# NightShade99/Self-Supervised-Vision

Hardware: AMD Instinct MI355X
Metric: images/sec (whole node) SimCLR ResNet-50 two-view train step (higher is better)
Workload: dtype f32; 1 GPU; SimCLR resnet50 (7x7/2 stem) synthetic 3x224x224, bs=512/GPU, global batch 512, NT-Xent(normalize, T=0.5) over the global batch, SGD-Nesterov; per_gpu_batch=512, global_batch=512, params=27971008, parallelism=single, view_streams=2, library=self-supervised-vision_amd/csrc/libssv_hip.so

## Files before the change

### include/ssv_hip.h

```cpp
#ifndef SSV_HIP_H
#define SSV_HIP_H

#include <stddef.h>
#include <stdint.h>

#ifdef __cplusplus
extern "C" {
#endif

typedef enum ssv_status {
  SSV_OK = 0,
  SSV_ERR_INVALID = -1,
  SSV_ERR_WORKSPACE = -2,
  SSV_ERR_LAUNCH = -3
} ssv_status;

int ssv_version(void);
const char* ssv_last_error(void);
const char* ssv_source_sha16(void);
int ssv_device_cus(void);

typedef struct ssv_conv_desc {
  int32_t N, H, W, C;
  int32_t K, R, S;
  int32_t stride, pad;
  int32_t Ho, Wo;
  int32_t arithmetic;
  int32_t reserved;
  const void* w_planes;
} ssv_conv_desc;
enum { SSV_ARITH_F32_MFMA = 0, SSV_ARITH_BF16X3 = 6 };
int ssv_conv_arithmetic(const ssv_conv_desc* d, int32_t product);
int ssv_split_planes(int64_t n, const float* x, void* planes, void* stream);

int ssv_conv2d_fwd(const ssv_conv_desc* d, const float* x, const float* w, const float* bias,
                   const float* addend, float* y, void* stream);
int ssv_pad_channels(int64_t npix, int32_t cin, int32_t cout, const float* in, float* out, int32_t accumulate, void* stream);
int ssv_group_expand(int32_t K, int32_t R, int32_t S, int32_t Cg, int32_t groups, const float* wg, float* wd, void* stream);
int ssv_group_extract(int32_t K, int32_t R, int32_t S, int32_t Cg, int32_t groups, const float* dwd, float* dwg, int32_t accumulate, void* stream);

int ssv_conv2d_fwd_grouped(const ssv_conv_desc* d, int32_t groups, const float* x, const float* wd, const float* bias, const float* addend,
                           float* y, void* stream);
int ssv_conv2d_dgrad_grouped(const ssv_conv_desc* d, int32_t groups, const float* dy, const float* wd, const float* addend, float* dx, void* stream);
size_t ssv_conv2d_wgrad_grouped_workspace_bytes(const ssv_conv_desc* d, int32_t groups);
int ssv_conv2d_wgrad_grouped(const ssv_conv_desc* d, int32_t groups, const float* x, const float* dy, float* dwd, int accumulate,
                             void* ws, size_t ws_bytes, void* stream);
int ssv_filter_transpose(int32_t K, int32_t R, int32_t S, int32_t C, const float* w, float* wt, void* stream);
int64_t ssv_conv2d_fwd_stats_groups(const ssv_conv_desc* d);
int ssv_conv2d_fwd_stats(const ssv_conv_desc* d, const float* x, const float* w, float* y, float* pmean, float* pm2, void* stream);
int ssv_conv2d_fwd_bnrelu_in_stats(const ssv_conv_desc* d, const float* x, const float* in_scale, const float* in_shift,
                                   const float* w, float* y, float* pmean, float* pm2, void* stream);
int ssv_conv2d_wgrad_bnrelu_in(const ssv_conv_desc* d, const float* x, const float* in_scale, const float* in_shift, const float* dy,
                               float* dw, int accumulate, void* ws, size_t ws_bytes, void* stream);
typedef struct ssv_bn_gate {
  const float* x;
  const float* scale;
  const float* shift;
  const uint8_t* mask;
  const float* mean;
  const float* invstd;
  float* psum_g;
  float* psum_gx;
  const float* x2;
  const float* mean2;
  const float* invstd2;
  float* psum_gx2;
} ssv_bn_gate;
int64_t ssv_conv2d_fwd_gate_groups(const ssv_conv_desc* d);
int ssv_conv2d_fwd_gated(const ssv_conv_desc* d, const float* x, const float* w, const float* addend, float* y,
                         const ssv_bn_gate* gate, void* stream);
typedef struct ssv_bn_dyin {
  const float* x;
  const float* coef;
} ssv_bn_dyin;
int ssv_conv2d_fwd_dyin(const ssv_conv_desc* d, const float* g, const ssv_bn_dyin* dyin, const float* w, const float* addend, float* y,
                        const ssv_bn_gate* gate, void* stream);
int ssv_conv2d_wgrad_dyin(const ssv_conv_desc* d, const float* x, const float* in_scale, const float* in_shift, const float* g,
                          const ssv_bn_dyin* dyin, float* dw, int accumulate, void* ws, size_t ws_bytes, void* stream);
int ssv_conv2d_fwd_sumin_stats(const ssv_conv_desc* d, const float* x, const float* res, const float* scale, const float* shift,
                               const float* rscale, const float* rshift, const float* w, float* y, float* pmean, float* pm2,
                               float* a_out, uint8_t* mask_out, void* stream);
int ssv_conv2d_fwd_gated_s2add(const ssv_conv_desc* d, const float* x, const float* w, const float* addend, int32_t H2, int32_t W2, float* y,
                               const ssv_bn_gate* gate, void* stream);
int ssv_conv2d_fwd_dyin_s2add(const ssv_conv_desc* d, const float* g, const ssv_bn_dyin* dyin, const float* w, const float* addend,
// ... 344 lines not shown
```

### self-supervised-vision_amd/csrc/conv_mfma.hip

```cpp
#include "common.h"
#include "split_bf16.h"
#include <string.h>
#include <type_traits>

namespace {

constexpr int GBK = 16;

__device__ __forceinline__ int xcd_remap(int orig, int nwg) {
  const int q = nwg >> 3, r = nwg & 7, xcd = orig & 7;
  return (xcd < r ? xcd * (q + 1) : r * (q + 1) + (xcd - r) * q) + (orig >> 3);
}

struct ConvKP {
  int N, H, W, C, K, R, S, stride, pad, Ho, Wo;
  int M;
  int RSC;
  FastDiv dHoWo, dWo, dC, dS, dWp;
  float* aux_out;
  float* aux_out2;
  const float* aux_in;
  const float* xf_scale;
  const float* xf_shift;
  ssv_bn_gate gate;
  const float* dyin_x;
  const float* dyin_coef;
  const float* sum_res; const float* sum_scale; const float* sum_shift; const float* sum_rscale; const float* sum_rshift;
  float* sum_out; uint8_t* sum_mask;
  long long bs_a, bs_b, bs_o;
  int add_H2, add_W2;
  int Cg, Kg;
  const unsigned short* w_planes;
  long long wp_stride;
};

__device__ __forceinline__ void group_span(int n0, int n1, int og, int ig, int bk, int ctot, int& lo, int& hi) {
  const int glo = n0 / og, ghi = (n1 - 1) / og;
  lo = glo * ig / bk * bk;
  hi = min(ctot, ((ghi + 1) * ig + bk - 1) / bk * bk);
}

constexpr int XF_MAXC = 1024;

__device__ __forceinline__ float gelu_f(float v) { return ssv_gelu(v); }
__device__ __forceinline__ float gelu_grad_f(float v) { return ssv_gelu_grad(v); }

using rsrc_t = __amdgpu_buffer_rsrc_t;
constexpr int OOB_OFF = (int)0x80000000u;
__device__ __forceinline__ rsrc_t make_rsrc(const void* base, unsigned bytes) {
  return __builtin_amdgcn_make_buffer_rsrc((void*)base, 0, bytes, 0x00020000);
}
__device__ __forceinline__ f32x4 bload4(rsrc_t rs, int voff_bytes, int soff_bytes) {
  typedef unsigned int u32x4_ __attribute__((ext_vector_type(4)));
  return __builtin_bit_cast(f32x4, (u32x4_)__builtin_amdgcn_raw_buffer_load_b128(rs, voff_bytes, soff_bytes, 0));
}

__device__ __forceinline__ int straddle_off(int off, int bytes, int& rot) {
  rot = 0;
  if (off == OOB_OFF) return OOB_OFF;
  if (off <= -16 || off >= bytes) return OOB_OFF;
  const int c = off < 0 ? 0 : (off > bytes - 16 ? bytes - 16 : off);
  rot = (off - c) >> 2;
  return c;
}
__device__ __forceinline__ f32x4 straddle_fix(f32x4 v, int rot) {
  f32x4 o;
#pragma unroll
  for (int e = 0; e < 4; ++e) {
    const int sidx = e + rot;
    float t = 0.f;
#pragma unroll
// ... 169 lines not shown
      for (int j = 0; j < TN16; ++j) lo[i][j] = f32x4{0.f, 0.f, 0.f, 0.f};
  }
  load_tile();
  xform_tile();
  store_tile();
  __syncthreads();
  for (int kt = 0; kt < nkt; ++kt) {
    load_tile();
    constexpr int TJ = TN16 / JSPLIT;
    static_assert(TN16 % JSPLIT == 0, "column tiles per group");
#pragma unroll
    for (int jg = 0; jg < JSPLIT; ++jg) {
      bf16x8 fb[TJ][3];
#pragma unroll
      for (int j = 0; j < TJ; ++j)
#pragma unroll
        for (int q = 0; q < 3; ++q) {
          if constexpr (KROWB) fb[j][q] = splitbf::krow_frag<RBB>(Bs + q * b_plane, wc0 + 16 * (jg * TJ + j), lane);
          else fb[j][q] = splitbf::rowk_frag(Bs + q * b_plane, wc0 + 16 * (jg * TJ + j), lane);
        }
#pragma unroll
      for (int i = 0; i < TM16; ++i) {
        bf16x8 fa[3];
#pragma unroll
        for (int q = 0; q < 3; ++q) {
          if constexpr (KROWA) fa[q] = splitbf::krow_frag<RBA>(As + q * a_plane, wr0 + 16 * i, lane);
          else fa[q] = splitbf::rowk_frag(As + q * a_plane, wr0 + 16 * i, lane);
        }
#pragma unroll
        for (int j = 0; j < TJ; ++j) {
          if constexpr (DUAL) splitbf::mma6x2(acc[i][jg * TJ + j], lo[i][jg * TJ + j], fb[j], fa);
          else splitbf::mma6(acc[i][jg * TJ + j], fb[j], fa);
        }
      }
    }
    if constexpr (FLUSH > 0) {
      if ((kt + 1) % FLUSH == 0) {
#pragma unroll
        for (int i = 0; i < TM16; ++i)
#pragma unroll
          for (int j = 0; j < TN16; ++j) { hi[i][j] += acc[i][j]; acc[i][j] = f32x4{0.f, 0.f, 0.f, 0.f}; }
      }
    }
    __syncthreads();
    if (kt + 1 < nkt) { xform_tile(); store_tile(); __syncthreads(); }
  }
#pragma unroll
  for (int i = 0; i < TM16; ++i)
#pragma unroll
    for (int j = 0; j < TN16; ++j) {
      if constexpr (FLUSH > 0) acc[i][j] = hi[i][j] + acc[i][j];
      if constexpr (DUAL) acc[i][j] += lo[i][j];
    }
}

__device__ __forceinline__ void bstore4(rsrc_t rs, int voff_bytes, f32x4 v) {
  typedef unsigned int u32x4_ __attribute__((ext_vector_type(4)));
  __builtin_amdgcn_raw_buffer_store_b128(__builtin_bit_cast(u32x4_, v), rs, voff_bytes, 0, 0);
}

struct SameOff {};
template <int TM, int TN>
__device__ __forceinline__ void stage_slab(const f32x16 (&acc)[TM][TN], float* __restrict__ ep, int tm, int lane) {
  constexpr int LDE = TN * 32 + 4;
  const int l31 = lane & 31, h = lane >> 5;
#pragma unroll
  for (int tn = 0; tn < TN; ++tn)
#pragma unroll
    for (int j = 0; j < 16; ++j) ep[((j & 3) + 8 * (j >> 2) + 4 * h) * LDE + tn * 32 + l31] = acc[tm][tn][j];
}
template <int TM, int TN>
__device__ __forceinline__ void stage_slab(const f32x4 (&acc)[2 * TM][2 * TN], float* __restrict__ ep, int tm, int lane) {
  constexpr int LDE = TN * 32 + 4;
  const int fr = lane & 15, kg = lane >> 4;
#pragma unroll
  for (int ii = 0; ii < 2; ++ii)
#pragma unroll
    for (int jj = 0; jj < 2 * TN; ++jj) *reinterpret_cast<f32x4*>(&ep[(16 * ii + fr) * LDE + 16 * jj + 4 * kg]) = acc[2 * tm + ii][jj];
}
template <bool SP, class A, class B> __device__ __forceinline__ auto& sel_acc(A& a, B& b) { if constexpr (SP) return b; else return a; }

template <int TM, int TN, int EPI = 0, bool STATS = false, int GATE = 0, class Acc, class RowOff, class AddOff = SameOff>
__device__ __forceinline__ void epilogue_vec(const Acc& acc, float* __restrict__ ep, int lane, int col0, int ncols,
                                             const float* __restrict__ bias, const float* addend, float* out, long long out_elems, RowOff&& row_off,
                                             float* out_act = nullptr, const float* gate = nullptr,
                                             float* pmean = nullptr, float* pm2 = nullptr, int group_rows = 0,
                                             const ssv_bn_gate* bn = nullptr, long long group = 0, AddOff add_off = AddOff(), long long add_elems = 0) {
  constexpr int LDE = TN * 32 + 4, C4 = TN * 8, RPI = 64 / C4, NP = 32 / RPI;
  constexpr bool GMASK = GATE >= 2, GX2 = GATE == 3;
  constexpr int HB0 = GATE == 1 ? 2 : 4;
  constexpr int HB = NP < HB0 ? NP : HB0;
  const int r_in = lane / C4, c4 = lane % C4;
  const int gcol = col0 + c4 * 4;
  const bool cok = gcol < ncols && r_in < RPI;
  const unsigned bytes = (unsigned)(out_elems * 4);
  const rsrc_t r_out = make_rsrc(out, bytes);
  f32x4 b4 = {0.f, 0.f, 0.f, 0.f};
  f32x4 st_p = {0.f, 0.f, 0.f, 0.f}, st_s1 = {0.f, 0.f, 0.f, 0.f}, st_s2 = {0.f, 0.f, 0.f, 0.f};
  f32x4 g_mu = {0.f, 0.f, 0.f, 0.f}, g_is = {0.f, 0.f, 0.f, 0.f}, g_sc = {0.f, 0.f, 0.f, 0.f}, g_sh = {0.f, 0.f, 0.f, 0.f};
  f32x4 g_mu2 = {0.f, 0.f, 0.f, 0.f}, g_is2 = {0.f, 0.f, 0.f, 0.f}, st_s3 = {0.f, 0.f, 0.f, 0.f};
  if constexpr (GATE != 0) {
    if (cok) {
      g_mu = *reinterpret_cast<const f32x4*>(bn->mean + gcol); g_is = *reinterpret_cast<const f32x4*>(bn->invstd + gcol);
      if constexpr (GATE == 1) { g_sc = *reinterpret_cast<const f32x4*>(bn->scale + gcol); g_sh = *reinterpret_cast<const f32x4*>(bn->shift + gcol); }
      if constexpr (GX2) { g_mu2 = *reinterpret_cast<const f32x4*>(bn->mean2 + gcol); g_is2 = *reinterpret_cast<const f32x4*>(bn->invstd2 + gcol); }
    }
// ... 86 lines not shown
          }
          bstore4(r_out, voff[sl][i], v);
          if constexpr (EPI == 1) {
            f32x4 a;
#pragma unroll
            for (int e = 0; e < 4; ++e) a[e] = gelu_f(v[e]);
            bstore4(r_act, voff[sl][i], a);
          }
        }
      };
      {
#pragma unroll
        for (int st = 0; st < NSTEP; ++st) {
          __builtin_amdgcn_sched_barrier(0);
          issue(st, 0);
          finish(st, 0);
        }
      }
    }
  };
  if constexpr (GATE != 0 || EPI == 2 || EPI == 5) rows(std::integral_constant<int, 2>{});
  else if (ADD) rows(std::integral_constant<int, 1>{});
  else rows(std::integral_constant<int, 0>{});

  if constexpr (STATS) {
#pragma unroll
    for (int o = C4; o < 64; o <<= 1) {
#pragma unroll
      for (int e = 0; e < 4; ++e) { st_s1[e] += __shfl_xor(st_s1[e], o, 64); st_s2[e] += __shfl_xor(st_s2[e], o, 64); }
    }
    if (r_in == 0 && cok && group_rows > 0) {
      const float n = (float)group_rows;
      *reinterpret_cast<f32x4*>(pmean + gcol) = st_p + st_s1 / n;
      *reinterpret_cast<f32x4*>(pm2 + gcol) = st_s2 - st_s1 * st_s1 / n;
    }
  }
  if constexpr (GATE != 0) {
#pragma unroll
    for (int o = C4; o < 64; o <<= 1) {
#pragma unroll
      for (int e = 0; e < 4; ++e) {
        st_s1[e] += __shfl_xor(st_s1[e], o, 64); st_s2[e] += __shfl_xor(st_s2[e], o, 64);
        if constexpr (GX2) st_s3[e] += __shfl_xor(st_s3[e], o, 64);
      }
    }
    if (r_in == 0 && cok) {
      *reinterpret_cast<f32x4*>(bn->psum_g + group * ncols + gcol) = st_s1;
      *reinterpret_cast<f32x4*>(bn->psum_gx + group * ncols + gcol) = st_s2;
      if constexpr (GX2) *reinterpret_cast<f32x4*>(bn->psum_gx2 + group * ncols + gcol) = st_s3;
    }
  }
}

template <int BM, int BN, int WGM, int WGN, int BK, bool VEC, int EPI = 0, bool STATS = false, int C4 = 0, bool XF = false, int GATE = 0, int OPM = 0, bool ADDS2 = false, int SP = 0>
__global__ void __launch_bounds__(256, (SP ? (OPM != 0 || GATE == 3 || (SP == 2 && BN == 128))
                                          : (OPM == 2 || GATE == 3 || (OPM == 1 && !(BM == 128 && BN == 128)))) ? 2 : 3)
conv_fwd_k(ConvKP p, const float* __restrict__ x, const float* __restrict__ w, const float* __restrict__ bias,
           const float* addend, float* y) {
  constexpr int TM = BM / WGM / 32, TN = BN / WGN / 32;
  constexpr int LDT = BK + 4;
  constexpr int STAGE = (BM + BN) * LDT;
  static_assert(!XF || (VEC && C4 == 0), "the fused-input variant is the float4 path");
  constexpr bool DYF = OPM == 1, SUM = OPM == 2;
  static_assert(OPM == 0 || (VEC && C4 == 0 && !XF), "the formed-on-load operands are the float4 path");
  constexpr int EP_FLOATS = 4 * 32 * (TN * 32 + 4);
  static_assert(!SP || (VEC && C4 == 0 && BK == 32), "the bf16-piece variants are the float4 path with K-step 32");
  constexpr int SP_FLOATS = (BM + BN) * 48;
  constexpr int SMEM = SP ? (SP_FLOATS > EP_FLOATS ? SP_FLOATS : EP_FLOATS)
                          : ((VEC && (EPI || STATS || GATE != 0 || OPM != 0) && EP_FLOATS > STAGE) ? EP_FLOATS : STAGE);
  __shared__ __attribute__((aligned(16))) float smem[SMEM];
  __shared__ __attribute__((aligned(16))) float xfs[(XF && !SP) ? 2 * XF_MAXC : 4];
  float* As = smem;
  float* Bs = smem + BM * LDT;
  const int tid = threadIdx.x, lane = tid & 63, wave = tid >> 6;
  const int wr0 = (wave / WGN) * (BM / WGM), wc0 = (wave % WGN) * (BN / WGN);
  const int NT = (p.K + BN - 1) / BN;
  const int bid = xcd_remap(blockIdx.x, gridDim.x);
  const int mt = bid / NT, nt = bid - mt * NT;
  const int m0 = mt * BM, n0 = nt * BN;
  x += (size_t)blockIdx.y * p.bs_a; w += (size_t)blockIdx.y * p.bs_b; y += (size_t)blockIdx.y * p.bs_o;
  if (addend) addend += (size_t)blockIdx.y * p.bs_o;

  f32x16 acc[SP ? 1 : TM][SP ? 1 : TN];
  f32x4 acc16[SP ? 2 * TM : 1][SP ? 2 * TN : 1];
  if constexpr (SP) {
#pragma unroll
    for (int i = 0; i < 2 * TM; ++i)
#pragma unroll
      for (int j = 0; j < 2 * TN; ++j) acc16[i][j] = f32x4{0.f, 0.f, 0.f, 0.f};
  } else zero_acc<SP ? 1 : TM, SP ? 1 : TN>(acc);

  if constexpr (VEC && C4 == 2) {
    static_assert(BK == 24 && BM == 256, "one staged output row per thread, six float4 per row");
    constexpr int CHN = BK / 4;
    constexpr int BF = (BN * CHN + 255) / 256;
    const rsrc_t rx = make_rsrc(x, (unsigned)p.N * p.H * p.W * 12u);
    const rsrc_t rw = make_rsrc(w, (unsigned)p.K * p.R * BK * 4u);
    int hi0, rowbase;
    unsigned wmask = 0;
    {
      const int m = m0 + tid;
      const bool ok = m < p.M;
      const uint32_t mm = ok ? (uint32_t)m : 0u;
      const uint32_t n = fdiv(mm, p.dHoWo);
      const uint32_t rem = mm - n * (uint32_t)(p.Ho * p.Wo);
      const uint32_t ho = fdiv(rem, p.dWo);
      const uint32_t wo = rem - ho * (uint32_t)p.Wo;
      hi0 = ok ? (int)ho * p.stride - p.pad : -(1 << 20);
      const int wi0 = (int)wo * p.stride - p.pad;
      rowbase = ok ? (((int)n * p.H + hi0) * p.W + wi0) * 12 : 0;
#pragma unroll
      for (int px = 0; px < 8; ++px) wmask |= (unsigned)((px < p.S) & ((unsigned)(wi0 + px) < (unsigned)p.W)) << px;
    }
    int boff[BF];
#pragma unroll
    for (int i = 0; i < BF; ++i) {
      const int f = tid + 256 * i, kf = f / CHN, ch = f - kf * CHN;
      boff[i] = (f < BN * CHN && n0 + kf < p.K) ? ((n0 + kf) * p.R * BK + ch * 4) * 4 : OOB_OFF;
    }
    int lr = 0;
// ... 34 lines not shown
      }
    };
    k_loop<TM, TN, true, true, LDT, LDT, BK, CHN + BF>(p.R, As, Bs, wr0, wc0, lane, acc, load_tile, store_tile, xform_tile);
  } else if constexpr (VEC && C4 == 1) {
    constexpr int CH = BK / 4, RPP = 256 / CH;
    constexpr int AP = BM / RPP, BP = BN / RPP;
    const int tl = tid % CH, rsub = tid / CH;
    const rsrc_t rx = make_rsrc(x, (unsigned)p.N * p.H * p.W * 16u);
    const rsrc_t rw = make_rsrc(w, (unsigned)p.K * p.RSC * 4u);
    int hi0[AP], wi0[AP], aoff[AP];
#pragma unroll
    for (int i = 0; i < AP; ++i) {
      const int m = m0 + rsub + RPP * i;
      const bool ok = m < p.M;
      const uint32_t mm = ok ? (uint32_t)m : 0u;
      const uint32_t n = fdiv(mm, p.dHoWo);
      const uint32_t rem = mm - n * (uint32_t)(p.Ho * p.Wo);
      const uint32_t ho = fdiv(rem, p.dWo);
      const uint32_t wo = rem - ho * (uint32_t)p.Wo;
      hi0[i] = ok ? (int)ho * p.stride - p.pad : -(1 << 20);
      wi0[i] = (int)wo * p.stride - p.pad;
      aoff[i] = (((int)n * p.H + hi0[i]) * p.W + wi0[i]) * 16;
    }
    int boff[BP];
#pragma unroll
    for (int i = 0; i < BP; ++i) {
      const int ko = n0 + rsub + RPP * i;
      boff[i] = ko < p.K ? ko * p.RSC * 4 : OOB_OFF;
    }
    const int ntap = p.R * p.S;
    int lt = tl;
    f32x4 ra[AP], rb[BP];
    auto load_tile = [&]() {
      const bool tv = lt < ntap;
      const int r = (int)fdiv((uint32_t)(tv ? lt : 0), p.dS);
      const int sx = (tv ? lt : 0) - r * p.S;
      const int toff_x = (r * p.W + sx) * 16, toff_w = lt * 16;
#pragma unroll
      for (int i = 0; i < AP; ++i) {
        const bool ok = tv & ((unsigned)(hi0[i] + r) < (unsigned)p.H) & ((unsigned)(wi0[i] + sx) < (unsigned)p.W);
        ra[i] = bload4(rx, ok ? aoff[i] + toff_x : OOB_OFF, 0);
      }
#pragma unroll
      for (int i = 0; i < BP; ++i) rb[i] = bload4(rw, (tv && boff[i] != OOB_OFF) ? boff[i] + toff_w : OOB_OFF, 0);
      lt += CH;
    };
    auto store_tile = [&]() {
#pragma unroll
      for (int i = 0; i < AP; ++i) *reinterpret_cast<f32x4*>(&As[(rsub + RPP * i) * LDT + tl * 4]) = ra[i];
#pragma unroll
      for (int i = 0; i < BP; ++i) *reinterpret_cast<f32x4*>(&Bs[(rsub + RPP * i) * LDT + tl * 4]) = rb[i];
    };
    k_loop<TM, TN, true, true, LDT, LDT, BK, AP + BP>((ntap + CH - 1) / CH, As, Bs, wr0, wc0, lane, acc, load_tile, store_tile);
  } else if constexpr (VEC) {
    constexpr int CH = BK / 4, RPP = 256 / CH;
    constexpr int AP = BM / RPP, BP = BN / RPP;
    const int chunk = (tid % CH) * 4, rsub = tid / CH;
    const rsrc_t rx = make_rsrc(x, (unsigned)p.N * p.H * p.W * p.C * 4u);
    const rsrc_t rw = make_rsrc(w, (unsigned)p.K * p.RSC * 4u);
    int hi0[AP], wi0[AP], aoff[AP];
#pragma unroll
    for (int i = 0; i < AP; ++i) {
      const int m = m0 + rsub + RPP * i;
      const bool ok = m < p.M;
      const uint32_t mm = ok ? (uint32_t)m : 0u;
      const uint32_t n = fdiv(mm, p.dHoWo);
      const uint32_t rem = mm - n * (uint32_t)(p.Ho * p.Wo);
      const uint32_t ho = fdiv(rem, p.dWo);
      const uint32_t wo = rem - ho * (uint32_t)p.Wo;
      hi0[i] = ok ? (int)ho * p.stride - p.pad : -(1 << 20);
      wi0[i] = (int)wo * p.stride - p.pad;
      aoff[i] = ((((int)n * p.H + hi0[i]) * p.W + wi0[i]) * p.C + chunk) * 4;
      if (!ok) aoff[i] = OOB_OFF;
    }
    int boff[BP];
#pragma unroll
    for (int i = 0; i < BP; ++i) {
      const int ko = n0 + rsub + RPP * i;
      boff[i] = ko < p.K ? (ko * p.RSC + chunk) * 4 : OOB_OFF;
    }
    const bool inb = p.pad == 0 && p.R == 1 && p.S == 1;
    int lr = 0, ls = 0, lc0 = 0;
    int ktiles = p.RSC / BK;
    if constexpr (!XF && OPM == 0) {
      if (p.Kg != 0) {
        int c_hi;
        group_span(n0, min(n0 + BN, p.K), p.Kg, p.Cg, BK, p.C, lc0, c_hi);
        ktiles = p.R * p.S * ((c_hi - lc0) / BK);
      }
    }
    f32x4 ra[AP], rb[SP ? 1 : BP];
    f32x4 ra2[OPM ? AP : 1], co[(OPM || (XF && SP)) ? 4 : 1];
    constexpr int BPP = SP ? (BN * 4 + 255) / 256 : 1;
    u32x4 rbp[SP ? 3 : 1][BPP];
    int boffp[BPP], bldsp[BPP];
    const long long wplane = p.wp_stride;
    const rsrc_t rwp = make_rsrc(SP ? (const void*)(p.w_planes + (size_t)blockIdx.y * p.bs_b) : (const void*)w, SP ? (unsigned)((2 * wplane + (long long)p.K * p.RSC) * 2) : 16u);
    if constexpr (SP) {
#pragma unroll
      for (int i = 0; i < BPP; ++i) {
        const int idx = tid + 256 * i, br = idx >> 2, k8 = idx & 3;
        boffp[i] = (idx < BN * 4 && n0 + br < p.K) ? ((n0 + br) * p.RSC + k8 * 8) * 2 : OOB_OFF;
        bldsp[i] = splitbf::rowk_off(br, k8);
      }
    }
    const rsrc_t rxs0 = make_rsrc((XF && SP) ? p.xf_scale : x, (XF && SP) ? (unsigned)p.C * 4u : 16u), rxs1 = make_rsrc((XF && SP) ? p.xf_shift : x, (XF && SP) ? (unsigned)p.C * 4u : 16u);
// ... 704 lines not shown
        const int row = i0 + wr0 + tm * 32 + (jj & 3) + 8 * (jj >> 2) + 4 * h;
        if (row < p.K) out[(size_t)row * p.RSC + col] = acc[tm][tn][jj];
      }
    }
  }
}

__global__ void __launch_bounds__(256)
wgrad_reduce_k(const float* __restrict__ partial, int nsplit, int64_t n, float* __restrict__ dw, int accumulate) {
  __shared__ float sm[4][64];
  const int e = threadIdx.x & 63, grp = threadIdx.x >> 6;
  const int64_t i = (int64_t)blockIdx.x * 64 + e;
  partial += (size_t)blockIdx.y * nsplit * n; dw += (size_t)blockIdx.y * n;
  const int per = (nsplit + 3) / 4;
  const int k0 = grp * per, k1 = min(k0 + per, nsplit);
  float s = 0.f;
  if (i < n) {
    int k = k0;
    for (; k + 3 < k1; k += 4) {
      const float a = partial[(size_t)k * n + i], b = partial[(size_t)(k + 1) * n + i];
      const float c = partial[(size_t)(k + 2) * n + i], d = partial[(size_t)(k + 3) * n + i];
      s += (a + b) + (c + d);
    }
    for (; k < k1; ++k) s += partial[(size_t)k * n + i];
  }
  sm[grp][e] = s;
  __syncthreads();
  if (grp == 0 && i < n) dw[i] = (accumulate ? dw[i] : 0.f) + ((sm[0][e] + sm[1][e]) + (sm[2][e] + sm[3][e]));
}

int check_desc(const ssv_conv_desc* d, const char* who) {
  SSV_REQUIRE(d != nullptr, "%s: null descriptor", who);
  SSV_REQUIRE(d->N > 0 && d->H > 0 && d->W > 0 && d->C > 0 && d->K > 0 && d->R > 0 && d->S > 0 && d->stride > 0 && d->pad >= 0,
              "%s: non-positive dimension", who);
  const int Ho = (d->H + 2 * d->pad - d->R) / d->stride + 1, Wo = (d->W + 2 * d->pad - d->S) / d->stride + 1;
  SSV_REQUIRE(Ho == d->Ho && Wo == d->Wo, "%s: Ho/Wo (%d,%d) inconsistent with input/filter/stride/pad (expect %d,%d)", who, d->Ho, d->Wo, Ho, Wo);
  SSV_REQUIRE((int64_t)d->N * d->H * d->W < (1ll << 31) && (int64_t)d->N * d->Ho * d->Wo < (1ll << 31), "%s: too many pixels", who);
  SSV_REQUIRE((int64_t)d->R * d->S * d->C < (1 << 24) && d->R * d->S <= 64 && d->H < 32768 && d->W < 32768, "%s: filter too large", who);
  SSV_REQUIRE((int64_t)d->N * d->H * d->W * d->C < (1ll << 29) - (1 << 22) && (int64_t)d->N * d->Ho * d->Wo * d->K < (1ll << 29) - (1 << 22) &&
              (int64_t)d->K * d->R * d->S * d->C < (1ll << 29), "%s: tensor of 2 GiB or more - split the batch", who);
  return SSV_OK;
}

ConvKP make_kp(const ssv_conv_desc* d) {
  ConvKP p;
  p.N = d->N; p.H = d->H; p.W = d->W; p.C = d->C; p.K = d->K; p.R = d->R; p.S = d->S;
  p.stride = d->stride; p.pad = d->pad; p.Ho = d->Ho; p.Wo = d->Wo;
  p.M = d->N * d->Ho * d->Wo;
  p.RSC = d->R * d->S * d->C;
  p.dHoWo = make_fastdiv((uint32_t)(d->Ho * d->Wo));
  p.dWo = make_fastdiv((uint32_t)d->Wo);
  p.dC = make_fastdiv((uint32_t)d->C);
  p.dS = make_fastdiv((uint32_t)d->S);
  p.dWp = make_fastdiv((uint32_t)d->W + 2u);
  p.aux_out = nullptr; p.aux_out2 = nullptr; p.aux_in = nullptr; p.xf_scale = nullptr; p.xf_shift = nullptr;
  memset(&p.gate, 0, sizeof(p.gate));
  p.dyin_x = nullptr; p.dyin_coef = nullptr;
  p.sum_res = p.sum_scale = p.sum_shift = p.sum_rscale = p.sum_rshift = nullptr; p.sum_out = nullptr; p.sum_mask = nullptr;
  p.bs_a = p.bs_b = p.bs_o = 0;
  p.add_H2 = p.add_W2 = 0;
  p.Cg = p.Kg = 0;
  p.w_planes = (const unsigned short*)d->w_planes;
  p.wp_stride = (long long)d->K * p.RSC;
  return p;
}

struct RowSplit { int nsplit, chunk; };
RowSplit wgrad_row_split(int bm, int64_t tiles, int64_t rows, int max_chunk = 0) {
  const int slots = bm == 128 ? 768 : 1024;
  int64_t ns = slots / tiles;
  const int64_t max_by_rows = cdiv64(rows, 256);
  if (ns > max_by_rows) ns = max_by_rows;
  if (ns < 1) ns = 1;
  int64_t chunk = cdiv64(cdiv64(rows, ns), 32) * 32;
  if (max_chunk > 0 && chunk > max_chunk) {
    const int64_t nb = cdiv64(rows, (int64_t)max_chunk);
    chunk = cdiv64(cdiv64(rows, nb), 32) * 32;
  }
  return {(int)cdiv64(rows, chunk), (int)chunk};
}

struct WgradPlan { int bm, bn, it, jt, nsplit, chunk; };
WgradPlan plan_wgrad(const ssv_conv_desc* d, int groups = 0) {
  WgradPlan w;
  const int RSC = d->R * d->S * d->C;
  const int64_t M = (int64_t)d->N * d->Ho * d->Wo;
  const bool bd = groups > 1 && d->C % 64 == 0;
  w.bm = (d->K >= 128 && !bd) ? 128 : 64;
  w.bn = (RSC <= 64 || bd) ? 64 : 128;
  w.it = cdiv(d->K, w.bm);
  w.jt = cdiv(RSC, w.bn);
  int tiles = w.it * w.jt;
  if (bd) {
    const int cg = d->C / groups, kg = d->K / groups;
    const int per_row = cdiv((cdiv(w.bm, kg) + 1) * cg, w.bn) + 1;
    tiles = w.it * d->R * d->S * (per_row < d->C / w.bn ? per_row : d->C / w.bn);
  }
  const RowSplit rs = wgrad_row_split(w.bm, tiles, M);
  w.chunk = rs.chunk; w.nsplit = rs.nsplit;
  return w;
}

}

namespace {

template <int V> using ic = std::integral_constant<int, V>;
template <int V0, int... Vs, class F>
inline void for_value(int v, F&& f) {
  if constexpr (sizeof...(Vs) == 0) f(ic<V0>{});
  else if (v == V0) f(ic<V0>{});
  else for_value<Vs...>(v, f);
}

inline bool sp_planes_fit(const ssv_conv_desc* d) {
  return (int64_t)d->K * d->R * d->S * d->C * 6 < (1ll << 31);
}
inline bool sp_fwd_ok(const ssv_conv_desc* d) {
  return d->arithmetic == SSV_ARITH_BF16X3 && d->w_planes != nullptr && (((uintptr_t)d->w_planes) & 15) == 0 && d->C % 32 == 0 && d->K % 4 == 0 &&
         sp_planes_fit(d);
}
constexpr int SP_DUAL_FROM = 1152;
inline int sp_fwd_mode(const ssv_conv_desc* d) {
  if (!sp_fwd_ok(d)) return 0;
  return (int64_t)d->R * d->S * d->C > SP_DUAL_FROM ? 2 : 1;
}
inline bool sp_dgrad_ok(const ssv_conv_desc* d) {
  return d->arithmetic == SSV_ARITH_BF16X3 && d->w_planes != nullptr && (((uintptr_t)d->w_planes) & 15) == 0 && d->K % 32 == 0 && d->C >= 128 && d->C % 8 == 0 &&
         sp_planes_fit(d);
}
inline bool sp_wgrad_ok(const ssv_conv_desc* d) {
  return d->arithmetic == SSV_ARITH_BF16X3 && d->C % 4 == 0 && d->K % 4 == 0;
}

struct FwdTile { int bm, bn, sp; unsigned grid_x; };
inline FwdTile fwd_tile(const ssv_conv_desc* d, int groups = 0) {
  FwdTile t;
  t.sp = sp_fwd_mode(d);
  const bool wide = d->K >= 128 && groups <= 1;
  t.bm = (wide || t.sp) ? 128 : 256;
  t.bn = wide ? 128 : 64;
  t.grid_x = (unsigned)(cdiv64((int64_t)d->N * d->Ho * d->Wo, t.bm) * cdiv(d->K, t.bn));
  return t;
}

enum { ARITH_ANY, ARITH_F32, ARITH_SPLIT };

struct FwdArgs { FwdTile t; unsigned batch; hipStream_t s; const ConvKP* p; const float* x; const float* w; const float* bias; const float* addend; float* y; };

template <int BK, int EPI = 0, bool STATS = false, int C4 = 0, bool XF = false, int GATE = 0, int OPM = 0, bool ADDS2 = false,
          int ARITH = (C4 != 0 || BK != 32) ? ARITH_F32 : ARITH_ANY>
inline void fwd_launch(const FwdArgs& a) {
  constexpr bool wide_only = ADDS2 || EPI != 0;
  auto arith = [&](auto SP) {
    auto tile = [&](auto BM, auto BN, auto WGM, auto WGN) {
      hipLaunchKernelGGL((conv_fwd_k<decltype(BM)::value, decltype(BN)::value, decltype(WGM)::value, decltype(WGN)::value, BK, true, EPI, STATS, C4, XF, GATE, OPM, ADDS2, decltype(SP)::value>),
                         dim3(a.t.grid_x, a.batch), dim3(256), 0, a.s, *a.p, a.x, a.w, a.bias, a.addend, a.y);
    };
    if (wide_only || a.t.bn == 128) tile(ic<128>{}, ic<128>{}, ic<2>{}, ic<2>{});
    else if constexpr (wide_only) {}
    else if constexpr (decltype(SP)::value != 0) tile(ic<128>{}, ic<64>{}, ic<2>{}, ic<2>{});
    else tile(ic<256>{}, ic<64>{}, ic<4>{}, ic<1>{});
  };
  if constexpr (ARITH == ARITH_F32) for_value<0>(a.t.sp, arith);
  else if constexpr (ARITH == ARITH_SPLIT) for_value<2, 1>(a.t.sp, arith);
  else for_value<2, 1, 0>(a.t.sp, arith);
}

int launch_fwd(const ssv_conv_desc* d, const float* x, const float* w, const float* bias, const float* addend, float* y,
               float* pmean, float* pm2, const float* in_scale, const float* in_shift, hipStream_t s, const ssv_bn_gate* gate = nullptr,
               int add_H2 = 0, int add_W2 = 0, int groups = 0) {
  ConvKP p = make_kp(d);
  p.add_H2 = add_H2; p.add_W2 = add_W2;
  p.aux_out = pmean; p.aux_out2 = pm2; p.xf_scale = in_scale; p.xf_shift = in_shift;
  if (groups > 1) { p.Cg = d->C / groups; p.Kg = d->K / groups; }
  if (gate) p.gate = *gate;
  const bool stats = pmean != nullptr, xf = in_scale != nullptr;
  const FwdArgs a = {fwd_tile(d, groups), 1, s, &p, x, w, bias, addend, y};
  if (gate) {
    const int gm = gate->x2 ? 3 : (gate->mask ? 2 : 1);
    if (add_H2 > 0) for_value<3, 2>(gm, [&](auto G) { fwd_launch<32, 0, false, 0, false, decltype(G)::value, 0, true>(a); });
    else for_value<3, 2, 1>(gm, [&](auto G) { fwd_launch<32, 0, false, 0, false, decltype(G)::value>(a); });
  }
  else if (stats && d->C == 4) fwd_launch<32, 0, true, 1>(a);
  else if (stats && xf) fwd_launch<32, 0, true, 0, true>(a);
  else if (stats) fwd_launch<32, 0, true>(a);
  else if (xf) fwd_launch<32, 0, false, 0, true>(a);
  else if (d->C == 4) fwd_launch<32, 0, false, 1>(a);
  else if (d->C % 32 == 0) fwd_launch<32>(a);
  else if (d->C % 16 == 0) fwd_launch<16>(a);
  else {
    const unsigned g2 = (unsigned)(cdiv(p.M, 128) * cdiv(d->K, 64));
    hipLaunchKernelGGL((conv_fwd_k<128, 64, 2, 2, GBK, false>), dim3(g2), dim3(256), 0, s, p, x, w, bias, addend, y);
  }
  return SSV_OK;
}

}

extern "C" int ssv_conv2d_fwd(const ssv_conv_desc* d, const float* x, const float* w, const float* bias,
                              const float* addend, float* y, void* stream) {
  if (int rc = check_desc(d, "ssv_conv2d_fwd")) return rc;
  SSV_REQUIRE(x && w && y, "ssv_conv2d_fwd: null pointer");
  SSV_REQUIRE((((uintptr_t)x | (uintptr_t)w | (uintptr_t)y) & 15) == 0, "ssv_conv2d_fwd: pointers must be 16-byte aligned");
  hipStream_t s = (hipStream_t)stream;
  ProfScope ps(SSV_PROF_CONV_FWD, s);
  launch_fwd(d, x, w, bias, addend, y, nullptr, nullptr, nullptr, nullptr, s);
  SSV_CHECK_LAUNCH("ssv_conv2d_fwd");
// ... 870 lines not shown
```

### self-supervised-vision_amd/ops.py

```python
import ctypes as C
import math
import os

import torch

from . import _lib
from ._lib import ConvDesc, call, ptr, stream, workspace

BN_EPS = 1e-5
BN_MOMENTUM = 0.1


def _empty(shape, like):
    return torch.empty(shape, dtype=torch.float32, device=like.device)


ARITHMETIC = os.environ.get("SSV_ARITHMETIC", "bf16x3")
if ARITHMETIC not in ("bf16x3", "f32"):
    raise _lib.SsvError(f"SSV_ARITHMETIC must be bf16x3 or f32 (got {ARITHMETIC!r})")


class arithmetic:

    def __init__(self, name):
        if name not in ("bf16x3", "f32"):
            raise _lib.SsvError(f"arithmetic must be bf16x3 or f32 (got {name!r})")
        self.name = name

    def __enter__(self):
        global ARITHMETIC
        self.prev, ARITHMETIC = ARITHMETIC, self.name
        invalidate_weight_caches()
        return self

    def __exit__(self, *exc):
        global ARITHMETIC
        ARITHMETIC = self.prev
        invalidate_weight_caches()
        return False


def conv_desc(x_shape, w_shape, stride, pad, w=None):
    n, h, w_, c = x_shape
    k, ci, r, s = w_shape
    if ci != c:
        raise _lib.SsvError(f"conv: input has {c} channels, filter expects {ci}")
    ho, wo = (h + 2 * pad - r) // stride + 1, (w_ + 2 * pad - s) // stride + 1
    d = ConvDesc(n, h, w_, c, k, r, s, stride, pad, ho, wo)
    if ARITHMETIC == "bf16x3":
        d.arithmetic = _lib.ARITH_BF16X3
        if w is not None and w.numel() % 8 == 0 and (c % 32 == 0 or k % 32 == 0):
            d.w_planes = ptr(_planes(w))
    return d


def _ohwi(w):
    if w.dim() == 2:
        if not w.is_contiguous():
            raise _lib.SsvError("linear weight must be contiguous")
        return w, (w.shape[0], w.shape[1], 1, 1)
    if not w.is_contiguous(memory_format=torch.channels_last):
        raise _lib.SsvError("conv filter must be in channels_last (OHWI) memory format")
    return w, tuple(w.shape)


_MAX_ELEMS = (1 << 29) - (1 << 22)


def _batch_chunks(n, per_sample_elems, rows_per_sample=None):
    worst = max(per_sample_elems)
    if n * worst < _MAX_ELEMS:
        return [(0, n)]
    nc = (_MAX_ELEMS - 1) // worst
    if nc < 1:
        raise _lib.SsvError("a single sample exceeds the 2 GiB per-launch tensor limit of the convolution kernels")
    if rows_per_sample is not None:
        q = 64 // math.gcd(rows_per_sample, 64)
        if nc // q * q < 1:
            raise _lib.SsvError(f"the statistics epilogue needs chunks of a multiple of {q} samples ({rows_per_sample} output rows per sample) but only "
                                f"{nc} sample(s) fit below the 2 GiB per-launch tensor limit: run this layer without the fused statistics "
                                f"(SSV_NO_BN_STATS_FUSION=1) or with smaller images")
        nc = nc // q * q
    return [(s0, min(s0 + nc, n)) for s0 in range(0, n, nc)]


def _sub(t, n0, n1):
    return None if t is None else t[n0:n1]


def conv2d_fwd(x, w, stride=1, pad=0, bias=None, addend=None, groups=1):
    _lib._dev(x, w, bias, addend)
    w, wshape = _ohwi(w)
    d = conv_desc(x.shape, wshape, stride, pad)
    y = _empty((d.N, d.Ho, d.Wo, d.K), x)
    for n0, n1 in _batch_chunks(d.N, (d.H * d.W * d.C, d.Ho * d.Wo * d.K)):
        dc = conv_desc((n1 - n0,) + tuple(x.shape[1:]), wshape, stride, pad, w=w)
        if groups > 1:
            call("ssv_conv2d_fwd_grouped", C.byref(dc), int(groups), ptr(x[n0:n1]), ptr(w), ptr(bias), ptr(_sub(addend, n0, n1)), ptr(y[n0:n1]), stream())
        else:
            call("ssv_conv2d_fwd", C.byref(dc), ptr(x[n0:n1]), ptr(w), ptr(bias), ptr(_sub(addend, n0, n1)), ptr(y[n0:n1]), stream())
    return y
# ... 1585 lines not shown
```

Baseline: 2952 images/sec.

## Stage 3x3 conv input as a shared strip reused across horizontal taps

Adds a strip-staged variant of the bf16x3 forward conv kernel for 3x3 stride-1 pad-1 convolutions with K<128. Per kernel row, the A tile is staged once into shared memory as a strip of pixel slots, and the three horizontal taps read shifted slot offsets from it. Before, each tap's im2col rows were loaded and split separately. This cuts global loads and bf16 splitting of the input by about 3x, at the cost of larger shared-memory use (152 slots), extra index arithmetic and more syncthreads per tap. A per-tap staging switch in Python keeps the old path available.

```diff
diff --git a/include/ssv_hip.h b/include/ssv_hip.h
--- a/include/ssv_hip.h
+++ b/include/ssv_hip.h
@@ -30,6 +30,7 @@
   const void* w_planes;
 } ssv_conv_desc;
 enum { SSV_ARITH_F32_MFMA = 0, SSV_ARITH_BF16X3 = 6 };
+enum { SSV_CONV_PER_TAP = 1 };
 int ssv_conv_arithmetic(const ssv_conv_desc* d, int32_t product);
 int ssv_split_planes(int64_t n, const float* x, void* planes, void* stream);
 
diff --git a/self-supervised-vision_amd/csrc/conv3x3_strip.h b/self-supervised-vision_amd/csrc/conv3x3_strip.h
--- /dev/null
+++ b/self-supervised-vision_amd/csrc/conv3x3_strip.h
@@ -0,0 +1,71 @@
+#pragma once
+#include <stdint.h>
+
+#if defined(__HIPCC__) || defined(__CUDACC__)
+#define SSV_STRIP_HD __host__ __device__ __forceinline__
+#else
+#define SSV_STRIP_HD inline
+#endif
+
+namespace strip3 {
+
+constexpr int MIN_W = 7;
+constexpr int max_slots(int bm, int w = MIN_W) { return bm + (bm + w - 1) / w + 2; }
+
+struct Div { uint32_t mul, shr, d; };
+inline Div make_div(uint32_t d) {
+  Div f; f.d = d ? d : 1;
+  if (f.d == 1) { f.mul = 0; f.shr = 0; return f; }
+  uint32_t lg = 31 - (uint32_t)__builtin_clz(f.d);
+  if (f.d & (f.d - 1)) lg += 1;
+  const uint32_t p = 31 + lg;
+  f.mul = (uint32_t)((((uint64_t)1 << p) + f.d - 1) / f.d);
+  f.shr = p - 32;
+  return f;
+}
+SSV_STRIP_HD uint32_t udiv(uint32_t n, const Div& f) { return f.d == 1 ? n : ((uint32_t)(((uint64_t)n * f.mul) >> 32) >> f.shr); }
+
+struct Plan { int H, W, M, a, g0; Div dW, dW1, dHW; };
+
+SSV_STRIP_HD Plan make_plan(int H, int W, int M, int m0, const Div& dW, const Div& dW1, const Div& dHW) {
+  Plan p;
+  p.H = H; p.W = W; p.M = M; p.dW = dW; p.dW1 = dW1; p.dHW = dHW;
+  p.g0 = (int)udiv((uint32_t)m0, dW);
+  p.a = m0 - p.g0 * W;
+  return p;
+}
+
+SSV_STRIP_HD int slot0(const Plan& p, int i) { return i + (int)udiv((uint32_t)(p.a + i), p.dW); }
+
+SSV_STRIP_HD int slots_used(const Plan& p, int bm) { return slot0(p, bm - 1) + 3; }
+
+SSV_STRIP_HD int slot_centre(const Plan& p, int j) {
+  const int t = j - 1 + p.a;
+  if (t < 0) return -1;
+  const int k = (int)udiv((uint32_t)t, p.dW1);
+  const int c = t - k * (p.W + 1);
+  if (c == p.W) return -1;
+  const int64_t pc = (int64_t)(p.g0 + k) * p.W + c;
+  return pc < p.M ? (int)pc : -1;
+}
+
+SSV_STRIP_HD int centre_row(const Plan& p, int pc) {
+  const uint32_t n = udiv((uint32_t)pc, p.dHW);
+  const uint32_t rem = (uint32_t)pc - n * (uint32_t)(p.H * p.W);
+  return (int)udiv(rem, p.dW);
+}
+
+SSV_STRIP_HD int slot_pixel(const Plan& p, int j, int r) {
+  const int pc = slot_centre(p, j);
+  if (pc < 0) return -1;
+  const int hi = centre_row(p, pc) + r - 1;
+  return (unsigned)hi < (unsigned)p.H ? pc + (r - 1) * p.W : -1;
+}
+
+constexpr int SLOT_BYTES = 64;
+SSV_STRIP_HD int piece_off(int slot, int piece) {
+  const int sg = ((piece & 1) << 1) | (piece >> 1);
+  return slot * SLOT_BYTES + ((sg ^ ((slot >> 2) & 1)) << 4);
+}
+
+}
diff --git a/self-supervised-vision_amd/csrc/conv_mfma.hip b/self-supervised-vision_amd/csrc/conv_mfma.hip
--- a/self-supervised-vision_amd/csrc/conv_mfma.hip
+++ b/self-supervised-vision_amd/csrc/conv_mfma.hip
@@ -1,5 +1,6 @@
 #include "common.h"
 #include "split_bf16.h"
+#include "conv3x3_strip.h"
 #include <string.h>
 #include <type_traits>
 
@@ -16,7 +17,7 @@
   int N, H, W, C, K, R, S, stride, pad, Ho, Wo;
   int M;
   int RSC;
-  FastDiv dHoWo, dWo, dC, dS, dWp;
+  FastDiv dHoWo, dWo, dC, dS, dW1;
   float* aux_out;
   float* aux_out2;
   const float* aux_in;
@@ -292,6 +293,58 @@
       if constexpr (FLUSH > 0) acc[i][j] = hi[i][j] + acc[i][j];
       if constexpr (DUAL) acc[i][j] += lo[i][j];
     }
+}
+
+template <int TM16, int TN16, bool DUAL, class LoadA, class LoadB, class StoreA, class StoreB, class Xform>
+__device__ __forceinline__ void k_loop_strip(int ngroups, const unsigned char* As, int a_plane, const unsigned char* Bs, int b_plane, const int (&arow)[TM16], int wc0, int lane,
+                                             f32x4 (&acc)[TM16][TN16], LoadA&& load_a, LoadB&& load_b, StoreA&& store_a, StoreB&& store_b, Xform&& xform_a) {
+  if (ngroups <= 0) return;
+  f32x4 lo[DUAL ? TM16 : 1][DUAL ? TN16 : 1];
+  if constexpr (DUAL) {
+#pragma unroll
+    for (int i = 0; i < TM16; ++i)
+#pragma unroll
+      for (int j = 0; j < TN16; ++j) lo[i][j] = f32x4{0.f, 0.f, 0.f, 0.f};
+  }
+  load_a();
+  load_b();
+  xform_a();
+  store_a();
+  store_b();
+  __syncthreads();
+  for (int g = 0; g < ngroups; ++g) {
+#pragma unroll
+    for (int s = 0; s < 3; ++s) {
+      if (s == 2) load_a();
+      load_b();
+      bf16x8 fb[TN16][3];
+#pragma unroll
+      for (int j = 0; j < TN16; ++j)
+#pragma unroll
+        for (int q = 0; q < 3; ++q) fb[j][q] = splitbf::rowk_frag(Bs + q * b_plane, wc0 + 16 * j, lane);
+#pragma unroll
+      for (int i = 0; i < TM16; ++i) {
+        bf16x8 fa[3];
+        const int off = strip3::piece_off(arow[i] + s, lane >> 4);
+#pragma unroll
+        for (int q = 0; q < 3; ++q) fa[q] = *reinterpret_cast<const bf16x8*>(As + q * a_plane + off);
+#pragma unroll
+        for (int j = 0; j < TN16; ++j) {
+          if constexpr (DUAL) splitbf::mma6x2(acc[i][j], lo[i][j], fb[j], fa);
+          else splitbf::mma6(acc[i][j], fb[j], fa);
+        }
+      }
+      __syncthreads();
+      if (s < 2) { store_b(); __syncthreads(); }
+      else if (g + 1 < ngroups) { xform_a(); store_a(); store_b(); __syncthreads(); }
+    }
+  }
+  if constexpr (DUAL) {
+#pragma unroll
+    for (int i = 0; i < TM16; ++i)
+#pragma unroll
+      for (int j = 0; j < TN16; ++j) acc[i][j] += lo[i][j];
+  }
 }
 
 __device__ __forceinline__ void bstore4(rsrc_t rs, int voff_bytes, f32x4 v) {
@@ -484,7 +537,7 @@
   }
 }
 
-template <int BM, int BN, int WGM, int WGN, int BK, bool VEC, int EPI = 0, bool STATS = false, int C4 = 0, bool XF = false, int GATE = 0, int OPM = 0, bool ADDS2 = false, int SP = 0>
+template <int BM, int BN, int WGM, int WGN, int BK, bool VEC, int EPI = 0, bool STATS = false, int C4 = 0, bool XF = false, int GATE = 0, int OPM = 0, bool ADDS2 = false, int SP = 0, bool STRIP = false>
 __global__ void __launch_bounds__(256, (SP ? (OPM != 0 || GATE == 3 || (SP == 2 && BN == 128))
                                           : (OPM == 2 || GATE == 3 || (OPM == 1 && !(BM == 128 && BN == 128)))) ? 2 : 3)
 conv_fwd_k(ConvKP p, const float* __restrict__ x, const float* __restrict__ w, const float* __restrict__ bias,
@@ -497,7 +550,10 @@
   static_assert(OPM == 0 || (VEC && C4 == 0 && !XF), "the formed-on-load operands are the float4 path");
   constexpr int EP_FLOATS = 4 * 32 * (TN * 32 + 4);
   static_assert(!SP || (VEC && C4 == 0 && BK == 32), "the bf16-piece variants are the float4 path with K-step 32");
-  constexpr int SP_FLOATS = (BM + BN) * 48;
+  static_assert(!STRIP || (SP && OPM == 0 && EPI == 0 && !ADDS2 && BM == 128), "the strip form: bf16 pieces, plain operand, 128-row tile");
+  constexpr int STRIP_SLOTS = 152;
+  static_assert(!STRIP || strip3::max_slots(BM) <= STRIP_SLOTS, "the static strip image holds the narrowest width the form accepts");
+  constexpr int SP_FLOATS = ((STRIP ? STRIP_SLOTS : BM) + BN) * 48;
   constexpr int SMEM = SP ? (SP_FLOATS > EP_FLOATS ? SP_FLOATS : EP_FLOATS)
                           : ((VEC && (EPI || STATS || GATE != 0 || OPM != 0) && EP_FLOATS > STAGE) ? EP_FLOATS : STAGE);
   __shared__ __attribute__((aligned(16))) float smem[SMEM];
@@ -638,6 +694,103 @@
       for (int i = 0; i < BP; ++i) *reinterpret_cast<f32x4*>(&Bs[(rsub + RPP * i) * LDT + tl * 4]) = rb[i];
     };
     k_loop<TM, TN, true, true, LDT, LDT, BK, AP + BP>((ntap + CH - 1) / CH, As, Bs, wr0, wc0, lane, acc, load_tile, store_tile);
+  } else if constexpr (VEC && STRIP) {
+    constexpr int SPP = 32;
+    constexpr int AP = (STRIP_SLOTS + SPP - 1) / SPP;
+    const int chunk = (tid & 7) * 4, rsub = tid >> 3;
+    const rsrc_t rx = make_rsrc(x, (unsigned)p.N * p.H * p.W * p.C * 4u);
+    const strip3::Plan sp = strip3::make_plan(p.H, p.W, p.M, m0, strip3::Div{p.dWo.mul, p.dWo.shr, p.dWo.d}, strip3::Div{p.dW1.mul, p.dW1.shr, p.dW1.d},
+                                              strip3::Div{p.dHoWo.mul, p.dHoWo.shr, p.dHoWo.d});
+    int hi0[AP], aoff[AP];
+#pragma unroll
+    for (int i = 0; i < AP; ++i) {
+      const int j = rsub + SPP * i;
+      const int pc = j < STRIP_SLOTS ? strip3::slot_centre(sp, j) : -1;
+      hi0[i] = pc >= 0 ? strip3::centre_row(sp, pc) - 1 : -(1 << 20);
+      aoff[i] = pc >= 0 ? ((pc - p.W) * p.C + chunk) * 4 : OOB_OFF;
+    }
+    int arow[2 * TM];
+#pragma unroll
+    for (int i = 0; i < 2 * TM; ++i) arow[i] = strip3::slot0(sp, wr0 + 16 * i + (lane & 15));
+    constexpr int BPP = (BN * 4 + 255) / 256;
+    u32x4 rbp[3][BPP];
+    int boffp[BPP], bldsp[BPP];
+    const long long wplane = p.wp_stride;
+    const rsrc_t rwp = make_rsrc((const void*)(p.w_planes + (size_t)blockIdx.y * p.bs_b), (unsigned)((2 * wplane + (long long)p.K * p.RSC) * 2));
+#pragma unroll
+    for (int i = 0; i < BPP; ++i) {
+      const int idx = tid + 256 * i, br = idx >> 2, k8 = idx & 3;
+      boffp[i] = (idx < BN * 4 && n0 + br < p.K) ? ((n0 + br) * p.RSC + k8 * 8) * 2 : OOB_OFF;
+      bldsp[i] = splitbf::rowk_off(br, k8);
+    }
+    const rsrc_t rxs0 = make_rsrc(XF ? p.xf_scale : x, XF ? (unsigned)p.C * 4u : 16u), rxs1 = make_rsrc(XF ? p.xf_shift : x, XF ? (unsigned)p.C * 4u : 16u);
+    f32x4 ra[AP], co[XF ? 2 : 1];
+    int xf_ok = 0;
+    int ar = 0, ac0 = 0;
+    int lr = 0, ls = 0, lc0 = 0;
+    auto load_a = [&]() {
+      const bool more = ac0 < p.C;
+      const int toff_x = (ar * p.W * p.C + ac0) * 4;
+      if constexpr (XF) { xf_ok = 0; co[0] = bload4(rxs0, chunk * 4, ac0 * 4); co[1] = bload4(rxs1, chunk * 4, ac0 * 4); }
+#pragma unroll
+      for (int i = 0; i < AP; ++i) {
+        const bool ok = more & ((unsigned)(hi0[i] + ar) < (unsigned)p.H);
+        ra[i] = bload4(rx, ok ? aoff[i] + toff_x : OOB_OFF, 0);
+        if constexpr (XF) xf_ok |= (int)ok << i;
+      }
+      ar += 1;
+      const bool w2 = ar == 3;
+      ar = w2 ? 0 : ar;
+      ac0 += w2 ? BK : 0;
+    };
+    auto load_b = [&]() {
+      const int toff_w = ((lr * 3 + ls) * p.C + lc0) * 4;
+#pragma unroll
+      for (int q = 0; q < 3; ++q)
+#pragma unroll
+        for (int i = 0; i < BPP; ++i)
+          rbp[q][i] = (u32x4)__builtin_amdgcn_raw_buffer_load_b128(rwp, boffp[i] == OOB_OFF ? OOB_OFF : boffp[i] + q * (int)(wplane * 2), toff_w >> 1, 0);
+      ls += 1;
+      const bool w1 = ls == 3;
+      ls = w1 ? 0 : ls;
+      lr += w1 ? 1 : 0;
+      const bool w2 = lr == 3;
+      lr = w2 ? 0 : lr;
+      lc0 += w2 ? BK : 0;
+    };
+    auto xform_a = [&]() {
+      if constexpr (XF) {
+#pragma unroll
+        for (int i = 0; i < AP; ++i) {
+          const float cap = ((xf_ok >> i) & 1) ? __builtin_inff() : 0.f;
+#pragma unroll
+          for (int e = 0; e < 4; ++e) ra[i][e] = __builtin_amdgcn_fmed3f(__builtin_fmaf(ra[i][e], co[0][e], co[1][e]), 0.f, cap);
+        }
+      }
+    };
+    constexpr int A_PLANE = STRIP_SLOTS * strip3::SLOT_BYTES, B_PLANE = BN * splitbf::ROWB;
+    unsigned char* const Asb = reinterpret_cast<unsigned char*>(smem);
+    unsigned char* const Bsb = Asb + 3 * A_PLANE;
+    auto store_a = [&]() {
+#pragma unroll
+      for (int i = 0; i < AP; ++i) {
+        if (STRIP_SLOTS % SPP == 0 || SPP * (i + 1) <= STRIP_SLOTS || rsub + SPP * i < STRIP_SLOTS) {
+          u32x2 pl[3];
+          splitbf::split4(ra[i], pl);
+          const int off = strip3::piece_off(rsub + SPP * i, (tid & 7) >> 1) + (tid & 1) * 8;
+#pragma unroll
+          for (int q = 0; q < 3; ++q) *reinterpret_cast<u32x2*>(Asb + q * A_PLANE + off) = pl[q];
+        }
+      }
+    };
+    auto store_b = [&]() {
+#pragma unroll
+      for (int q = 0; q < 3; ++q)
+#pragma unroll
+        for (int i = 0; i < BPP; ++i)
+          if (BN * 4 % 256 == 0 || tid + 256 * i < BN * 4) *reinterpret_cast<u32x4*>(Bsb + q * B_PLANE + bldsp[i]) = rbp[q][i];
+    };
+    k_loop_strip<2 * TM, 2 * TN, SP == 2>(3 * (p.C / BK), Asb, A_PLANE, Bsb, B_PLANE, arow, wc0, lane, acc16, load_a, load_b, store_a, store_b, xform_a);
   } else if constexpr (VEC) {
     constexpr int CH = BK / 4, RPP = 256 / CH;
     constexpr int AP = BM / RPP, BP = BN / RPP;
@@ -1448,7 +1601,7 @@
   p.dWo = make_fastdiv((uint32_t)d->Wo);
   p.dC = make_fastdiv((uint32_t)d->C);
   p.dS = make_fastdiv((uint32_t)d->S);
-  p.dWp = make_fastdiv((uint32_t)d->W + 2u);
+  p.dW1 = make_fastdiv((uint32_t)d->W + 1u);
   p.aux_out = nullptr; p.aux_out2 = nullptr; p.aux_in = nullptr; p.xf_scale = nullptr; p.xf_shift = nullptr;
   memset(&p.gate, 0, sizeof(p.gate));
   p.dyin_x = nullptr; p.dyin_coef = nullptr;
@@ -1521,6 +1674,10 @@
   if (!sp_fwd_ok(d)) return 0;
   return (int64_t)d->R * d->S * d->C > SP_DUAL_FROM ? 2 : 1;
 }
+inline bool sp_fwd_strip(const ssv_conv_desc* d, int groups = 0) {
+  return sp_fwd_ok(d) && d->R == 3 && d->S == 3 && d->stride == 1 && d->pad == 1 && groups <= 1 && d->K < 128 && d->W >= strip3::MIN_W &&
+         !(d->reserved & SSV_CONV_PER_TAP);
+}
 inline bool sp_dgrad_ok(const ssv_conv_desc* d) {
   return d->arithmetic == SSV_ARITH_BF16X3 && d->w_planes != nullptr && (((uintptr_t)d->w_planes) & 15) == 0 && d->K % 32 == 0 && d->C >= 128 && d->C % 8 == 0 &&
          sp_planes_fit(d);
@@ -1529,10 +1686,11 @@
   return d->arithmetic == SSV_ARITH_BF16X3 && d->C % 4 == 0 && d->K % 4 == 0;
 }
 
-struct FwdTile { int bm, bn, sp; unsigned grid_x; };
+struct FwdTile { int bm, bn, sp; unsigned grid_x; bool strip; };
 inline FwdTile fwd_tile(const ssv_conv_desc* d, int groups = 0) {
   FwdTile t;
   t.sp = sp_fwd_mode(d);
+  t.strip = sp_fwd_strip(d, groups);
   const bool wide = d->K >= 128 && groups <= 1;
   t.bm = (wide || t.sp) ? 128 : 256;
   t.bn = wide ? 128 : 64;
@@ -1548,8 +1706,16 @@
           int ARITH = (C4 != 0 || BK != 32) ? ARITH_F32 : ARITH_ANY>
 inline void fwd_launch(const FwdArgs& a) {
   constexpr bool wide_only = ADDS2 || EPI != 0;
+  constexpr bool has_strip = BK == 32 && C4 == 0 && OPM == 0 && EPI == 0 && !ADDS2;
   auto arith = [&](auto SP) {
     auto tile = [&](auto BM, auto BN, auto WGM, auto WGN) {
+      if constexpr (has_strip && decltype(SP)::value != 0 && decltype(BN)::value == 64) {
+        if (a.t.strip) {
+          hipLaunchKernelGGL((conv_fwd_k<decltype(BM)::value, decltype(BN)::value, decltype(WGM)::value, decltype(WGN)::value, BK, true, EPI, STATS, C4, XF, GATE, OPM, ADDS2, decltype(SP)::value, true>),
+                             dim3(a.t.grid_x, a.batch), dim3(256), 0, a.s, *a.p, a.x, a.w, a.bias, a.addend, a.y);
+          return;
+        }
+      }
       hipLaunchKernelGGL((conv_fwd_k<decltype(BM)::value, decltype(BN)::value, decltype(WGM)::value, decltype(WGN)::value, BK, true, EPI, STATS, C4, XF, GATE, OPM, ADDS2, decltype(SP)::value>),
                          dim3(a.t.grid_x, a.batch), dim3(256), 0, a.s, *a.p, a.x, a.w, a.bias, a.addend, a.y);
     };
diff --git a/self-supervised-vision_amd/ops.py b/self-supervised-vision_amd/ops.py
--- a/self-supervised-vision_amd/ops.py
+++ b/self-supervised-vision_amd/ops.py
@@ -37,6 +37,25 @@
         global ARITHMETIC
         ARITHMETIC = self.prev
         invalidate_weight_caches()
+        return False
+
+
+PER_TAP_STAGING = False
+
+
+class per_tap_staging:
+
+    def __init__(self, on=True):
+        self.on = bool(on)
+
+    def __enter__(self):
+        global PER_TAP_STAGING
+        self.prev, PER_TAP_STAGING = PER_TAP_STAGING, self.on
+        return self
+
+    def __exit__(self, *exc):
+        global PER_TAP_STAGING
+        PER_TAP_STAGING = self.prev
         return False
 
 
@@ -47,6 +66,7 @@
         raise _lib.SsvError(f"conv: input has {c} channels, filter expects {ci}")
     ho, wo = (h + 2 * pad - r) // stride + 1, (w_ + 2 * pad - s) // stride + 1
     d = ConvDesc(n, h, w_, c, k, r, s, stride, pad, ho, wo)
+    d.reserved = 1 if PER_TAP_STAGING else 0
     if ARITHMETIC == "bf16x3":
         d.arithmetic = _lib.ARITH_BF16X3
         if w is not None and w.numel() % 8 == 0 and (c % 32 == 0 or k % 32 == 0):
```

Result: no change. 2946 images/sec, median of 2 (-0.2%).
